# CSB5/lofreq

Measured on AMD Instinct MI355X. Metric: pileup columns/sec at depth 10000, higher is better.
Workload: dtype f64

## Files before the change

lofreq_amd/csrc/lfq_api.hip:

```cpp
#include "lfq_bound.h"
#include "lfq_ctx.h"

namespace {

struct LfqDeviceStreams {
    hipStream_t stream = nullptr, dps = nullptr, side[2] = {nullptr, nullptr};
    hipEvent_t ev_tail[3] = {nullptr, nullptr, nullptr};
    bool tail_recorded = false;
    hipEvent_t ev_end = nullptr;
    bool end_recorded = false;
    int refs = 0;
};
std::mutex g_streams_m;
LfqDeviceStreams g_streams[64];

bool acquire_streams(int device, lfq_ctx *c);
void release_streams(int device);

void *pin_acquire_impl(lfq_ctx *c, size_t bytes, int *slot)
{
    int best = -1, empty = -1, smallest = -1;
    for (int i = 0; i < LFQ_PIN_SLOTS; i++) {
        auto &b = c->pin_pool[i];
        if (b.used) {
// ... 576 lines not shown
                                   (LFQ_MAX_SEGMENTS + 1) * LFQ_NCOUNTERS * sizeof(int32_t), hipMemcpyDeviceToHost, st));
        LFQ_TRY_HIP(hipEventRecord(c->ev[3], st));
        c->batch_recorded = 1;
        return LFQ_OK;
    }

    int64_t max_depth = tr->max_col_obs;
    if (max_depth <= 0) {
        LFQ_TRY(lfq_launch_maxdepth(T, gcounters, st));
        LFQ_TRY_HIP(hipMemcpyAsync(c->h_counters, gcounters, LFQ_NCOUNTERS * sizeof(int32_t), hipMemcpyDeviceToHost, st));
        LFQ_TRY_HIP(hipStreamSynchronize(st));
        max_depth = c->h_counters[LFQ_GC_MAXDEPTH];
    }
    {
        static const LfqLuts h_luts = [] {
            LfqLuts h;
            fill_luts(&h);
            return h;
        }();
        const bool lb = !P.general && P.def_alt_bq == 0 && P.def_alt_jp < 0.0;
        P.bound_p_lo = (lb && !indel_mode && kn.bound_gate && lfq_count_is_lean(T, P, max_depth))
                           ? lfq_bound_p_lo(h_luts.bq, P.min_alt_bq4, LFQ_BOUND_QLO) : 0.0;
    }
    const int64_t per_block = 3 * max_depth + 72;
    int n_big_blocks = c->n_cu;
    const int64_t budget = (int64_t)1 << 29;
    if (per_block * n_big_blocks > budget) {
        n_big_blocks = (int)std::max<int64_t>(8, budget / per_block);
    }
    LFQ_TRY(grow(&c->d_scratch, &c->scratch_doubles, per_block * n_big_blocks));
    if (!c->d_longs) {
        c->long_cap = 1 << 16;
        c->pool_cells = kn.split_pool_cells;
        LFQ_TRY_HIP(hipMalloc((void **)&c->d_longs, (size_t)c->long_cap * sizeof(LfqLong)));
        LFQ_TRY_HIP(hipMalloc((void **)&c->d_pool, (size_t)std::max(c->pool_cells, 1) * sizeof(LfqSegCell)));
        LFQ_TRY_HIP(hipEventCreateWithFlags(&c->ev_segw, hipEventDisableTiming));
        LFQ_TRY_HIP(hipEventCreateWithFlags(&c->ev_prep, hipEventDisableTiming));
        LFQ_TRY_HIP(hipEventCreateWithFlags(&c->ev_mid, hipEventDisableTiming));
    }

    const int n_seg = 1;
    c->cur_segments = n_seg;
    LFQ_TRY_HIP(hipEventRecord(c->ev_join[2], st));
    LFQ_TRY_HIP(hipStreamWaitEvent(dps, c->ev_join[2], 0));

    bool big_joined = false;
    for (int s = 0; s < n_seg; s++) {
        const int64_t c0 = ncols * s / n_seg, c1 = ncols * (s + 1) / n_seg;
        LfqWork W;
        W.tested_prefix = c->d_prefix;
        W.entries = c->d_entries + c0;
        W.counters = c->d_counters + s * LFQ_NCOUNTERS;
        W.gcounters = gcounters;
        W.block_sums = (int32_t *)(c->d_tiles + 2 * (c0 / 1024 + 8 * s));
        W.long_cap = c->long_cap / n_seg;
        W.pool_cells = c->pool_cells / n_seg;
        W.longs = c->d_longs + (int64_t)s * W.long_cap;
        W.pool = c->d_pool + (int64_t)s * W.pool_cells;
        W.unsplit = c->d_unsplit + c0;

        LFQ_TRY_HIP(hipEventRecord(c->ev_cnt[s][0], st));
        const bool ungated = c->batch_gate == LFQ_GATE_NONE && st == c->stream && !c->priv_stream_on && !single_stream;
        LFQ_TRY(lfq_launch_count(T, c0, c1, P, c->d_luts, d_counts, c->d_flags, max_depth, st, ungated));
        c->cur_sparse_counts = P.sparse_counts && lfq_count_is_shallow(T, P, max_depth);
        LFQ_TRY_HIP(hipEventRecord(c->ev_cnt[s][1], st));

        LFQ_TRY_HIP(hipStreamWaitEvent(dps, c->ev_cnt[s][1], 0));
        LFQ_TRY(lfq_launch_scan(T, c0, c1, c->d_flags, d_counts, W, dps));
        if (P.approx_n > 0) {
            LFQ_TRY(grow(&c->d_approx_mu, &c->approx_mu_bytes, (c1 - c0) * 8));
            LFQ_TRY(lfq_launch_approx_gate(T, P, c->d_luts, d_counts, W, c1 - c0, (double *)c->d_approx_mu, c->d_flags, dps));
            LFQ_TRY(lfq_launch_scan(T, c0, c1, c->d_flags, d_counts, W, dps, true));
        }
        LFQ_TRY_HIP(hipEventRecord(c->ev_scan[s], dps));
        const bool sb_heavy = n_seg == 1 && !indel_mode && c->leader && !kn.no_sb_precompute;
        auto launch_heavy = [&]() -> int {
            if (P.lazy_strand) {
                LFQ_TRY(lfq_launch_strand_heavy(T, W, d_counts, c->d_tuples_mapped, c->d_nheavy_mapped, c->heavy_cap, 16, dps));
            } else {
                LFQ_TRY(lfq_launch_gather_heavy(W, d_counts, c->d_tuples_mapped, c->d_nheavy_mapped, c->heavy_cap, 16, dps));
            }
            LFQ_TRY_HIP(hipEventRecord(c->ev_heavy, dps));
            {
                std::lock_guard<std::mutex> lk(*c->lm);
                c->leader_go++;
                c->sb_pending++;
            }
            c->lcv->notify_all();
            return LFQ_OK;
        };
        const bool screen = !kn.skip_light && kn.light_kernel != 2;
        if (sb_heavy && !screen) {
            LFQ_TRY(launch_heavy());
        }
        const int64_t seg_cols = c1 - c0;
        const int screen_auto = (c->batch_gate == LFQ_GATE_NONE && !indel_mode) ? (tr->max_col_obs >= 4096 ? 1 : 2) : 4;
        const int light_waves_per_cu = kn.light_kernel == 0 ? screen_auto : 10;
        const int n_light_waves = (int)std::min<int64_t>((int64_t)c->n_cu * light_waves_per_cu, std::max<int64_t>(seg_cols / 8, 4));
        const int n_mid_waves = (int)std::min<int64_t>((int64_t)c->n_cu * 4, std::max<int64_t>(seg_cols, 4));
        const bool run_big = !kn.skip_big, run_mid = !kn.skip_mid;
        const bool dbg_sync = kn.debug_sync != 0;
#define LFQ_DBG_STAGE(name)                                                        \
    do {                                                                           \
        if (dbg_sync) {                                                            \
            fprintf(stderr, "[lfq] %s launched\n", name);                          \
            hipError_t e_ = hipDeviceSynchronize();                                \
            fprintf(stderr, "[lfq] %s done (%d)\n", name, (int)e_);                \
        }                                                                          \
    } while (0)
        LFQ_TRY_HIP(hipStreamWaitEvent(side1, c->ev_scan[s], 0));
        LFQ_TRY_HIP(hipEventRecord(c->ev_side[1][s][0], side1));
        LFQ_TRY_HIP(hipStreamWaitEvent(side0, c->ev_scan[s], 0));
        LFQ_TRY_HIP(hipEventRecord(c->ev_side[0][s][0], side0));
        if (run_big) {
            LFQ_TRY(lfq_launch_dp_big_prep(T, P, c->d_luts, d_counts, W, d_pvals, pvals_capacity, c->n_cu * 2, side0));
            LFQ_DBG_STAGE("prep");
        }
        LFQ_TRY_HIP(hipEventRecord(c->ev_prep, side0));
        if (run_mid) {
            LFQ_TRY(lfq_launch_dp_mid(T, P, c->d_luts, d_counts, W, d_pvals, pvals_capacity, n_mid_waves, side1));
            LFQ_DBG_STAGE("mid");
        }
        const bool big_on_st = run_big && !single_stream && !kn.big_on_side && c->batch_gate != LFQ_GATE_NONE;
        if (big_on_st) {
            LFQ_TRY_HIP(hipStreamWaitEvent(st, c->ev_prep, 0));
            LFQ_TRY(lfq_launch_dp_big(T, P, c->d_luts, d_counts, W, d_pvals, pvals_capacity, c->d_scratch, per_block,
                                      n_big_blocks, st));
            LFQ_DBG_STAGE("big");
            LFQ_TRY_HIP(hipEventRecord(c->ev_segw, st));
            big_joined = true;
        }
        if (run_big) {
            LFQ_TRY(lfq_launch_dp_seg(1, T, P, c->d_luts, W, c->n_cu * 8, side0));
            LFQ_DBG_STAGE("seg big");
            LFQ_TRY(tail_record(c, 0, side0));
            LFQ_TRY(lfq_launch_dp_combine(1, P, d_counts, W, d_pvals, pvals_capacity, c->n_cu, side0));
            LFQ_DBG_STAGE("combine big");
            if (!big_on_st) {
                LFQ_TRY(lfq_launch_dp_big(T, P, c->d_luts, d_counts, W, d_pvals, pvals_capacity, c->d_scratch, per_block,
                                          n_big_blocks, side0));
                LFQ_DBG_STAGE("big");
            }
        }
        if (!run_big) {
            LFQ_TRY(tail_record(c, 0, side0));
        }
        LFQ_TRY_HIP(hipStreamWaitEvent(side1, c->ev_prep, 0));
        if (run_mid || run_big) {
            LFQ_TRY(lfq_launch_dp_seg(0, T, P, c->d_luts, W, c->n_cu * 8, side1));
            LFQ_DBG_STAGE("seg mid");
            LFQ_TRY(tail_record(c, 1, side1));
            LFQ_TRY(lfq_launch_dp_combine(0, P, d_counts, W, d_pvals, pvals_capacity, c->n_cu, side1));
            LFQ_DBG_STAGE("combine mid");
        }
        if (!(run_mid || run_big)) {
            LFQ_TRY(tail_record(c, 1, side1));
        }
        LFQ_TRY_HIP(hipEventRecord(c->ev_light[s][0], dps));
        if (!kn.skip_light) {
            if (kn.light_kernel == 2) {
                LFQ_TRY(lfq_launch_dp_light(T, P, c->d_luts, d_counts, W, d_pvals, pvals_capacity, n_light_waves, dps));
            } else {
                const int kh = indel_mode ? c->kreg_hint_indel : c->kreg_hint;
                LFQ_TRY(lfq_launch_dp_quad(T, P, c->d_luts, d_counts, W, c->d_retry + c0, d_pvals, pvals_capacity,
                                           n_light_waves, kh, dps, 1));
                LFQ_TRY(tail_record(c, 2, dps));
                if (sb_heavy) {
                    LFQ_TRY(launch_heavy());
                }
                LFQ_TRY(lfq_launch_dp_quad(T, P, c->d_luts, d_counts, W, c->d_retry + c0, d_pvals, pvals_capacity,
                                           n_light_waves, kh, dps, 2));
            }
        }
        LFQ_TRY_HIP(hipEventRecord(c->ev_light[s][1], dps));
        if (!screen) {
            LFQ_TRY(tail_record(c, 2, dps));
        }
        for (int i = 0; i < 2; i++) {
            LFQ_TRY_HIP(hipEventRecord(c->ev_side[i][s][1], side_i[i]));
        }
    }
    hipStream_t jn = (st != c->stream || single_stream) ? st : side0;
// ... 760 lines not shown
```

lofreq_amd/csrc/lfq_dp.hip:

```cpp
#include <atomic>

#include "lfq_bound.h"
#include "lfq_device.h"

#define LFQ_LN2_HI 6.93147180369123816490e-01
#define LFQ_LN2_LO 1.90821492927058770002e-10
#define LFQ_EXP_UNDERFLOW_X (-708.3964185322641)
#define LFQ_DBL_EPS 2.220446049250313e-16

#ifndef LFQ_HEAVY_WAVES
#define LFQ_HEAVY_WAVES 8
#endif
#ifndef LFQ_DP512_WAVES
#define LFQ_DP512_WAVES 2
#endif

struct LfqColCtx {
    int col;
    uint64_t off0;
    int64_t n_obs;
    int ref_code;
    int median_ref_bq;
    int K;
    int64_t bonf;
// ... 363 lines not shown
template <int C>
__device__ __forceinline__ void lfq_strip_store_cells(const LfqStrip<C> &S, int gl, int shift, int K, LfqSegCell *out)
{
#pragma unroll
    for (int j = 0; j < C; j++) {
        const int k = gl * C + j - shift;
        if (k >= 0 && k <= K && (k < K || j == 0)) {
            const double v = S.v[j];
            LfqSegCell c;
            c.v = (v > 0.0) ? __builtin_amdgcn_frexp_mant(v) : 0.0;
            c.e = (v > 0.0) ? S.e + __builtin_amdgcn_frexp_exp(v) : LFQ_EXT_ZERO_E;
            c.pad_ = 0;
            out[k] = c;
        }
    }
}

__device__ __forceinline__ int lfq_split_plan(int K, int64_t rem_chunks, int phase1, int seg_max)
{
    if (K > LFQ_SPLIT_MAX_K) {
        return 0;
    }
    int64_t n_new = seg_max - phase1;
    n_new = min(n_new, rem_chunks / (rem_chunks < LFQ_SEG_SHORT_BELOW ? LFQ_SEG_MIN_CHUNKS_SHORT : LFQ_SEG_MIN_CHUNKS));
    n_new = min(n_new, max(rem_chunks * 64 / (2 * (int64_t)max(K, 1)) + 1 - phase1, (int64_t)3 - phase1));
    return n_new >= 2 ? (int)n_new : 0;
}

__device__ __forceinline__ int lfq_seg_class(int K)
{
    return K <= 63 ? 0 : (K <= 252 ? 1 : (K <= 504 ? 2 : (K <= 1008 ? 3 : 4)));
}

__device__ __forceinline__ LfqLong *lfq_long_reserve(const LfqWork &W, int K, int n_seg, int64_t *cell0)
{
    const int cells = 2 * n_seg * (K + 1);
    const int c0 = atomicAdd(&W.counters[LFQ_CNT_POOL], cells);
    if (c0 + cells > W.pool_cells) {
        return nullptr;
    }
    const int cls = lfq_seg_class(K);
    const int per_class = W.long_cap / LFQ_SEG_CLASSES;
    const int slot = atomicAdd(&W.counters[LFQ_CNT_LONG0 + cls], 1);
    if (slot >= per_class) {
        return nullptr;
    }
    *cell0 = c0;
    return W.longs + cls * per_class + slot;
}

__device__ __forceinline__ void lfq_ctx_from_long(LfqColCtx &cx, const LfqLong &r, const LfqParams &P)
{
    cx.col = r.col;
    cx.off0 = r.off0;
    cx.n_obs = r.n_obs;
    cx.ref_code = r.ref_code;
    cx.median_ref_bq = r.median_ref_bq;
    cx.K = r.K;
    cx.bonf = r.bonf;
    cx.bonf_d = (double)r.bonf;
    cx.sig_s = P.sig * (1.0 + P.prune_slack);
    if (r.force_fe) {
        cx.sig_s = fmax(cx.sig_s, 4.5e-16 * cx.bonf_d);
    }
}

__device__ __forceinline__ void lfq_seg_range(const LfqLong &rec, int r, int64_t *c0, int64_t *c1)
{
    const int64_t n_chunks = ((int64_t)rec.n_obs + 63) / 64;
    const int64_t rem = n_chunks - rec.ch_begin;
    const int n_new = rec.n_seg - rec.phase1;
    *c0 = rec.ch_begin + rem * (r - rec.phase1) / n_new;
    *c1 = rec.ch_begin + rem * (r - rec.phase1 + 1) / n_new;
}

__device__ __forceinline__ double lfq_logaddexp(double a, double b)
{
    const double hi = fmax(a, b), lo = fmin(a, b);
    if (lo == -INFINITY) {
// ... 281 lines not shown
            }
            if (pf.want_entry) {
                *pf.entry = lfq_load_entry(pf.entry_ptr, 0);
            }
        }
        if (PREFETCH && ch + 1 < n_chunks) {
            raw = lfq_load_chunk(cx, ch + 1, T);
        }
#ifdef LFQ_PROFILE
        const long long c2 = clock64();
        t_load += c2 - c1;
#endif
        const bool hit = lfq_strip_chunk2<C>(S, reinterpret_cast<const LfqRow2 *>(rows), tflag, lt, cx.bonf_d, cx.sig_s);
#ifdef LFQ_PROFILE
        t_rows += clock64() - c2;
#endif
        n_rows += __popcll(S.rows >= 64 ? km : (km & ((1ull << S.rows) - 1ull)));
        if (hit) {
            pruned = true;
            break;
        }
        if (SPLIT && ch + 1 == P.phase1_chunks) {
            const int n_new = lfq_split_plan(K, n_chunks - (ch + 1), 1,
                                             min(P.seg_max_mid, max(2, P.seg_budget_mid / max(W.counters[LFQ_CNT_MID], 1))));
            if (n_new > 0) {
                const int n_seg = n_new + 1;
                const int cells = 2 * n_seg * (K + 1);
                const int cls = lfq_seg_class(K);
                const int per_class = W.long_cap / LFQ_SEG_CLASSES;
                const int c0 = lfq_claim(&W.counters[LFQ_CNT_POOL], cells);
                if (c0 + cells <= W.pool_cells) {
                    const int slot = lfq_claim(&W.counters[LFQ_CNT_LONG0 + cls], 1);
                    if (slot < per_class) {
                        lfq_strip_store_cells<C>(S, lane, shift, K, W.pool + c0);
                        if (lane == 0) {
                            LfqLong r;
                            r.off0 = cx.off0;
                            r.bonf = cx.bonf;
                            r.cell0 = c0;
                            r.n_obs = (int32_t)cx.n_obs;
                            r.col = cx.col;
                            r.K = K;
                            r.n_seg = n_seg;
                            r.ch_begin = (int32_t)(ch + 1);
                            r.phase1 = 1;
                            r.uf_mask = 0;
                            r.force_fe = 0;
                            r.pruned = 0;
                            r.rows = n_rows;
                            r.median_ref_bq = (int16_t)cx.median_ref_bq;
                            r.ref_code = (uint8_t)cx.ref_code;
                            r.pad0_ = 0;
                            r.pad1_ = 0;
                            r.uf_bound[0] = r.uf_bound[1] = r.uf_bound[2] = 0.0;
                            r.pad_[0] = r.pad_[1] = r.pad_[2] = r.pad_[3] = 0;
                            W.longs[cls * per_class + slot] = r;
                        }
                        return;
                    }
                }
            }
        }
        if (!PREFETCH && ch + 1 < n_chunks) {
            raw = lfq_load_chunk(cx, ch + 1, T);
        }
    }
#ifdef LFQ_PROFILE
    if (lane == 0) {
        atomicAdd(&W.counters[8], (int)(t_stage >> 8));
        atomicAdd(&W.counters[9], (int)(t_load >> 8));
        atomicAdd(&W.counters[10], (int)(t_rows >> 8));
        atomicAdd(&W.counters[11], n_rows);
    }
#endif
#ifdef LFQ_TRACE
    if (lane == 0) printf("col %d K %d C %d: rows done pruned=%d n_rows=%d\n", cx.col, K, C, (int)pruned, n_rows);
#endif
    if (lane == 0) {
        lfq_account(W, n_rows, K);
    }
    if (!pruned && !lfq_strip_final_prune<C>(S, lt, cx.bonf_d, cx.sig_s)) {
#ifdef LFQ_TRACE
        if (lane == 0) printf("col %d: emitting\n", cx.col);
#endif
        const lfq_col_counts cnt = counts[cx.col];
        S.rows = n_rows;
        lfq_emit_linear<C>(cx, cnt, S, shift, lt, W, pvals, pvals_capacity);
    }
}

template <int MAXC>
__global__ __launch_bounds__(256) void lfq_dp_wave_kernel(LfqTracksDev T, LfqParams P,
                                                          const LfqLuts *__restrict__ g_luts,
                                                          const lfq_col_counts *__restrict__ counts, LfqWork W,
                                                          int base_idx, int count_idx,
                                                          lfq_col_pvals *__restrict__ pvals,
                                                          int64_t pvals_capacity, int batch, int only_if_gl64)
{
    __shared__ LfqLuts s_luts;
    __shared__ LfqRow s_rows[4][64];
    (void)only_if_gl64;
    if (MAXC > 1) {
        __builtin_amdgcn_s_setprio(3);
    }
    lfq_luts_to_lds(&s_luts, g_luts);
    __syncthreads();
    const int wave = __builtin_amdgcn_readfirstlane((int)(threadIdx.x >> 6));
    const int n_work = W.counters[count_idx];
    const LfqEntry *list = W.entries + ((base_idx >= 0) ? W.counters[base_idx] : 0);
    LfqRow *rows = s_rows[wave];

    const int BATCH = batch;
    int32_t *head = &W.counters[(MAXC == 1) ? LFQ_CNT_HEAD_LIGHT : LFQ_CNT_HEAD_MID];
    for (;;) {
        int b0 = lfq_claim(head, BATCH);
        if (b0 >= n_work) {
            break;
        }
        const int b1 = min(b0 + BATCH, n_work);
        int w = b0;
        LfqEntry en = lfq_load_entry(list, w);
        LfqRaw raw = lfq_load_chunk_at(en.off0, en.n_obs, 0, T);
        LfqEntry en_next = en;
        bool have_next = (w + 1) < b1;
        if (have_next) {
            en_next = lfq_load_entry(list, w + 1);
        }
        for (;;) {
            LfqColCtx cx;
            lfq_col_setup(cx, en, P);
            LfqRaw raw_next = raw;
            LfqEntry en_next2 = en_next;
            const bool have_next2 = have_next && (w + 2) < b1;
            LfqPrefetch pf;
            pf.want_raw = have_next;
            pf.off0 = en_next.off0;
            pf.n_obs = en_next.n_obs;
            pf.want_entry = have_next2;
            pf.entry_ptr = list + (have_next2 ? (w + 2) : w);
            pf.raw = &raw_next;
            pf.entry = &en_next2;
            if (MAXC == 1 || cx.K < 64) {
                lfq_wave_column<1, (MAXC > 1), (MAXC > 1)>(cx, raw, T, P, &s_luts, rows, counts, W, pvals, pvals_capacity, pf);
            } else {
                lfq_wave_column<4, true, true>(cx, raw, T, P, &s_luts, rows, counts, W, pvals, pvals_capacity, pf);
            }
            if (!have_next) {
                break;
// ... 611 lines not shown
                                                 LfqSegCell *out)
{
    const int lane = lfq_lane();
    const int K = cx.K;
    const int shift = (C - K % C) % C;
    const int lt = (K + shift) / C;
    const double tflag = (lane == lt) ? 1.0 : 0.0;
    LfqStrip<C> S;
    lfq_strip_init<C>(S, true, shift);
    bool pruned = false;
    int n_rows = 0;
    LfqRaw raw = lfq_load_chunk(cx, ch0, T);
    for (int64_t ch = ch0; ch < ch1; ch++) {
        const uint64_t km = lfq_stage_rows2(cx, raw, P, L, reinterpret_cast<LfqRow2 *>(rows));
        if (ch + 1 < ch1) {
            raw = lfq_load_chunk(cx, ch + 1, T);
        }
        const bool hit = lfq_strip_chunk2<C>(S, reinterpret_cast<const LfqRow2 *>(rows), tflag, lt, cx.bonf_d, cx.sig_s);
        n_rows += __popcll(S.rows >= 64 ? km : (km & ((1ull << S.rows) - 1ull)));
        if (hit) {
            pruned = true;
            break;
        }
    }
    if (!pruned && lfq_strip_final_prune<C>(S, lt, cx.bonf_d, cx.sig_s)) {
        pruned = true;
    }
    lfq_strip_store_cells<C>(S, lane, shift, K, out);
    if (lane == 0) {
        __builtin_nontemporal_store(n_rows | (pruned ? (int)0x40000000 : 0), &out[0].pad_);
    }
}

template <int MODE>
__global__ __launch_bounds__(256) void lfq_dp_seg_kernel(LfqTracksDev T, LfqParams P,
                                                         const LfqLuts *__restrict__ g_luts, LfqWork W)
{
    __shared__ LfqLuts s_luts;
    __shared__ LfqRow s_rows[4][64];
    __builtin_amdgcn_s_setprio(3);
    lfq_luts_to_lds(&s_luts, g_luts);
    __syncthreads();
    constexpr int C_LO = MODE ? 2 : 0, C_N = MODE ? 3 : 2;
    const int wave = __builtin_amdgcn_readfirstlane((int)(threadIdx.x >> 6));
    const int per_class = W.long_cap / LFQ_SEG_CLASSES;
    int n_items[C_N], total = 0;
#pragma unroll
    for (int c = 0; c < C_N; c++) {
        n_items[c] = min(W.counters[LFQ_CNT_LONG0 + C_LO + c], per_class) * LFQ_SEG_MAX;
        total += n_items[c];
    }
    LfqRow *rows = s_rows[wave];
    const int n_waves_total = (int)gridDim.x * 4;
    for (int idx = (int)blockIdx.x * 4 + wave; idx < total; idx += n_waves_total) {
        int c = 0, i = idx;
#pragma unroll
        for (int k = 0; k < C_N - 1; k++) {
            if (c == k && i >= n_items[k]) {
                i -= n_items[k];
                c = k + 1;
            }
        }
        const int r = i % LFQ_SEG_MAX;
        const LfqLong R = W.longs[(C_LO + c) * per_class + i / LFQ_SEG_MAX];
        if (r < R.phase1 || r >= R.n_seg) {
            continue;
        }
        LfqColCtx cx;
        lfq_ctx_from_long(cx, R, P);
        int64_t c0, c1;
        lfq_seg_range(R, r, &c0, &c1);
        LfqSegCell *out = W.pool + R.cell0 + (int64_t)r * (R.K + 1);
        if (MODE == 0) {
            if (c == 0) {
                lfq_wave_segment<1>(cx, c0, c1, T, P, &s_luts, rows, out);
            } else {
                lfq_wave_segment<4>(cx, c0, c1, T, P, &s_luts, rows, out);
            }
        } else {
            if (c == 0) {
                lfq_wave_segment<8>(cx, c0, c1, T, P, &s_luts, rows, out);
            } else if (c == 1) {
                lfq_wave_segment<16>(cx, c0, c1, T, P, &s_luts, rows, out);
            } else {
                lfq_wave_segment<32>(cx, c0, c1, T, P, &s_luts, rows, out);
            }
        }
    }
}


#ifndef LFQ_COMB_THREADS
#define LFQ_COMB_THREADS 512
#endif
#define LFQ_FOLD_MAX_CLASS 3
#define LFQ_COMB_CELLS 2048
#define LFQ_COMB_PER_THREAD (LFQ_COMB_CELLS / LFQ_COMB_THREADS)

struct LfqCombShared {
    double av[LFQ_COMB_CELLS];
// ... 894 lines not shown
        atomicAdd(&W.gcounters[LFQ_GC_APPROX_PRUNED], 1);
    }
}

int lfq_launch_approx_gate(const LfqTracksDev &t, const LfqParams &p, const LfqLuts *d_luts, const lfq_col_counts *d_counts,
                           const LfqWork &w, int64_t ncols_seg, double *d_mu, uint8_t *d_flags, void *stream)
{
    if (ncols_seg <= 0) {
        return LFQ_OK;
    }
    const unsigned waves = (unsigned)std::min<int64_t>(ncols_seg, 256 * 32);
    hipLaunchKernelGGL(lfq_approx_mu_kernel, dim3((waves + 3) / 4), dim3(256), 0, (hipStream_t)stream, t, p, d_luts, d_counts,
                       w, d_mu);
    hipLaunchKernelGGL(lfq_approx_gate_kernel, dim3((unsigned)((ncols_seg + 255) / 256)), dim3(256), 0, (hipStream_t)stream,
                       p, w, (const double *)d_mu, d_flags);
    return hipGetLastError() == hipSuccess ? LFQ_OK : LFQ_ERR_HIP;
}

int lfq_launch_dp_light(const LfqTracksDev &t, const LfqParams &p, const LfqLuts *d_luts,
                        const lfq_col_counts *d_counts, const LfqWork &w, lfq_col_pvals *d_pvals,
                        int64_t pvals_capacity, int n_waves, void *stream)
{
    if (t.ncols <= 0 || n_waves <= 0) {
        return LFQ_OK;
    }
    const unsigned blocks = (unsigned)((n_waves + 3) / 4);
    hipLaunchKernelGGL(lfq_dp_wave_kernel<1>, dim3(blocks), dim3(256), 0, (hipStream_t)stream, t, p, d_luts,
                       d_counts, w, -1, LFQ_CNT_LIGHT, d_pvals, pvals_capacity, 32, 0);
    return hipGetLastError() == hipSuccess ? LFQ_OK : LFQ_ERR_HIP;
}

int lfq_launch_dp_mid(const LfqTracksDev &t, const LfqParams &p, const LfqLuts *d_luts,
                      const lfq_col_counts *d_counts, const LfqWork &w, lfq_col_pvals *d_pvals,
                      int64_t pvals_capacity, int n_waves, void *stream)
{
    if (t.ncols <= 0 || n_waves <= 0) {
        return LFQ_OK;
    }
    const unsigned blocks = (unsigned)((n_waves + 3) / 4);
    hipLaunchKernelGGL(lfq_dp_wave_kernel<4>, dim3(blocks), dim3(256), 0, (hipStream_t)stream, t, p,
                       d_luts, d_counts, w, LFQ_CNT_LIGHT, LFQ_CNT_MID, d_pvals, pvals_capacity, 1, 0);
    return hipGetLastError() == hipSuccess ? LFQ_OK : LFQ_ERR_HIP;
}

int lfq_launch_dp_big(const LfqTracksDev &t, const LfqParams &p, const LfqLuts *d_luts,
                      const lfq_col_counts *d_counts, const LfqWork &w, lfq_col_pvals *d_pvals,
                      int64_t pvals_capacity, double *d_scratch, int64_t scratch_doubles_per_block,
                      int n_blocks, void *stream)
{
    if (t.ncols <= 0 || n_blocks <= 0) {
        return LFQ_OK;
    }
    hipLaunchKernelGGL(lfq_dp_big_kernel, dim3((unsigned)n_blocks), dim3(LFQ_HEAVY_WAVES * 64), 0,
                       (hipStream_t)stream, t, p, d_luts, d_counts, w, d_pvals, pvals_capacity, d_scratch,
                       scratch_doubles_per_block);
    return hipGetLastError() == hipSuccess ? LFQ_OK : LFQ_ERR_HIP;
}


int lfq_launch_dp_big_prep(const LfqTracksDev &t, const LfqParams &p, const LfqLuts *d_luts,
                           const lfq_col_counts *d_counts, const LfqWork &w, lfq_col_pvals *d_pvals,
                           int64_t pvals_capacity, int n_blocks, void *stream)
{
    if (t.ncols <= 0 || n_blocks <= 0) {
        return LFQ_OK;
    }
    hipLaunchKernelGGL(lfq_dp_big_prep_kernel, dim3((unsigned)n_blocks), dim3(LFQ_PREP_WAVES * 64), 0,
                       (hipStream_t)stream, t, p, d_luts, d_counts, w, d_pvals, pvals_capacity);
    return hipGetLastError() == hipSuccess ? LFQ_OK : LFQ_ERR_HIP;
}

int lfq_launch_dp_seg(int mode, const LfqTracksDev &t, const LfqParams &p, const LfqLuts *d_luts,
                      const LfqWork &w, int n_waves, void *stream)
{
    if (t.ncols <= 0 || n_waves <= 0) {
        return LFQ_OK;
    }
    const dim3 grid((unsigned)((n_waves + 3) / 4)), block(256);
    if (mode == 0) {
        hipLaunchKernelGGL(lfq_dp_seg_kernel<0>, grid, block, 0, (hipStream_t)stream, t, p, d_luts, w);
    } else {
        hipLaunchKernelGGL(lfq_dp_seg_kernel<1>, grid, block, 0, (hipStream_t)stream, t, p, d_luts, w);
    }
    return hipGetLastError() == hipSuccess ? LFQ_OK : LFQ_ERR_HIP;
}

int lfq_launch_dp_combine(int mode, const LfqParams &p, const lfq_col_counts *d_counts, const LfqWork &w,
                          lfq_col_pvals *d_pvals, int64_t pvals_capacity, int n_blocks, void *stream)
{
    if (n_blocks <= 0) {
        return LFQ_OK;
    }
    {
        static std::atomic<unsigned long long> allowed{0ull};
        int dev = 0;
        if (hipGetDevice(&dev) != hipSuccess) {
            return LFQ_ERR_HIP;
        }
        const unsigned long long bit = 1ull << (dev & 63);
        if (!(allowed.load(std::memory_order_acquire) & bit)) {
            const int bytes = (int)sizeof(LfqCombShared);
            if (hipFuncSetAttribute(reinterpret_cast<const void *>(&lfq_dp_combine_kernel<0>),
                                    hipFuncAttributeMaxDynamicSharedMemorySize, bytes) != hipSuccess ||
                hipFuncSetAttribute(reinterpret_cast<const void *>(&lfq_dp_combine_kernel<1>),
                                    hipFuncAttributeMaxDynamicSharedMemorySize, bytes) != hipSuccess) {
                return LFQ_ERR_HIP;
            }
            allowed.fetch_or(bit, std::memory_order_release);
        }
    }
    if (mode == 0) {
        hipLaunchKernelGGL(lfq_dp_fold_kernel<0>, dim3((unsigned)n_blocks * 4), dim3(64 * LFQ_FOLD_WAVES), 0,
                           (hipStream_t)stream, p, d_counts, w, d_pvals, pvals_capacity);
        hipLaunchKernelGGL(lfq_dp_combine_kernel<0>, dim3((unsigned)n_blocks), dim3(LFQ_COMB_THREADS), sizeof(LfqCombShared),
                           (hipStream_t)stream, p, d_counts, w, d_pvals, pvals_capacity, 1);
    } else {
// ... 57 lines not shown
```

lofreq_amd/csrc/lfq_host.cpp:

```cpp
#include <errno.h>
#include <fenv.h>
#include <float.h>
#include <limits.h>
#include <math.h>
#include <stdio.h>
#include <stdlib.h>
#include <string.h>

#include <algorithm>
#include <atomic>
#include <chrono>
#include <condition_variable>
#include <functional>
#include <mutex>
#include <sched.h>
#include <string>
#include <thread>
#include <unordered_map>
#include <vector>

#include "lofreq_amd.h"
#include "lfq_internal.h"

#ifdef LFQ_TUNE
// ... 23 lines not shown
        x.host_loop_threads = geti("LFQ_HOST_LOOP_THREADS", 8);
        x.host_spin_us = geti("LFQ_HOST_SPIN_US", 2000);
        x.local_world_size = (int)std::max(1L, geti("LOCAL_WORLD_SIZE", 1));
        x.no_sb_precompute = LFQ_TUNE_HAS("LFQ_NO_SB_PRECOMPUTE");
#ifdef LFQ_TUNE
        if (const char *sk = getenv("LFQ_DEBUG_SKIP")) {
            x.skip_light = strstr(sk, "light") != nullptr;
            x.skip_mid = strstr(sk, "mid") != nullptr;
            x.skip_big = strstr(sk, "big") != nullptr;
        }
        if (const char *lk = getenv("LFQ_LIGHT_KERNEL")) {
            x.light_kernel = !strcmp(lk, "wave") ? 2 : 0;
        }
#endif
        x.screen_rounds = (int)std::max(1L, LFQ_TUNE_I("LFQ_SCREEN_ROUNDS", 24));
        {
            const long both = LFQ_TUNE_I("LFQ_SEG_MAX", -1);
            const long big = LFQ_TUNE_I("LFQ_SEG_MAX_BIG", both), mid = LFQ_TUNE_I("LFQ_SEG_MAX_MID", both);
            x.seg_max = big < 0 ? -1 : (int)std::min((long)LFQ_SEG_MAX, std::max(2L, big));
            x.seg_max_mid = mid < 0 ? -1 : (int)std::min((long)LFQ_SEG_MAX, std::max(2L, mid));
        }
        x.split_pool_cells = (int)std::max(0L, LFQ_TUNE_I("LFQ_SPLIT_POOL_CELLS", 8L << 20));
        x.count_multi_below = LFQ_TUNE_I("LFQ_COUNT_MULTI_BELOW", 4096);
        x.big_on_side = LFQ_TUNE_HAS("LFQ_BIG_ON_SIDE");
        x.pileup_tiles = (int)LFQ_TUNE_I("LFQ_PILEUP_TILES", 1);
        x.baq_one_variant = LFQ_TUNE_HAS("LFQ_BAQ_ONE_VARIANT") ? 1 : 0;
        x.count_lpg4_below = LFQ_TUNE_I("LFQ_COUNT_LPG4_BELOW", 320);
        x.count_lpg8_below = LFQ_TUNE_I("LFQ_COUNT_LPG8_BELOW", 900);
        x.host_par_min = std::max(1L, LFQ_TUNE_I("LFQ_HOST_PAR_MIN", 200000));
        x.indel_host_pack = LFQ_TUNE_HAS("LFQ_INDEL_HOST_PACK");
        x.pileup_atomic = LFQ_TUNE_HAS("LFQ_PILEUP_ATOMIC");
        x.baq_lds = LFQ_TUNE_I("LFQ_BAQ_LDS", 1) != 0;
        x.bound_gate = LFQ_TUNE_I("LFQ_BOUND_GATE", 1) != 0;
        (void)geti;
        (void)has;
        return x;
    }();
    return k;
}

namespace {

inline double phred_to_prob(int q)
{
    return (q == INT_MAX) ? DBL_MIN : pow(10.0, -1.0 * q / 10.0);
}

inline int prob_to_phred(long double p) { return (int)(-10.0 * log10l(p)); }

inline int prob_to_phred_safe(double p) { return (p <= 0.0) ? INT_MAX : (int)(-10.0 * log10l(p)); }

inline int eps_cmp(double a, double b)
{
    if (fabs(a - b) < DBL_EPSILON) {
        return 0;
    }
    return a < b ? -1 : (a > b ? 1 : 0);
}

struct IndexedP {
    double p;
    int64_t i;
};

void sort_indexed(std::vector<IndexedP> &v)
{
// ... 1268 lines not shown
```

lofreq_amd/csrc/lfq_internal.h:

```cpp
#ifndef LFQ_INTERNAL_H
#define LFQ_INTERNAL_H

#include <stdint.h>

#include "lofreq_amd.h"

struct LfqLuts {
    double bq[256];
    double baq[256];
    double mq[256];
    double sq[256];
};

struct LfqParams {
    int32_t min_bq4;
    int32_t min_alt_bq4;
    int32_t def_alt_bq;
    int32_t general;
    double jq_reject_above;
    double alt_jq_reject_above;
    double def_alt_jp;
    int32_t min_cov;
    int32_t use_baq, use_mq, use_sq;
    int32_t bonf_dynamic;
// ... 36 lines not shown
    int32_t pad2_;
};

#define LFQ_FLAG_NLO_SHIFT 3

struct LfqSegCell {
    double v;
    int32_t e;
    int32_t pad_;
};

struct LfqLong {
    uint64_t off0;
    int64_t bonf;
    int64_t cell0;
    int32_t n_obs, col;
    int32_t K;
    int32_t n_seg;
    int32_t ch_begin;
    int32_t phase1;
    uint32_t uf_mask;
    int32_t force_fe;
    int32_t pruned;
    int32_t rows;
    int16_t median_ref_bq;
    uint8_t ref_code;
    uint8_t pad0_;
    int32_t pad1_;
    double uf_bound[3];
    int64_t pad_[4];
};

#define LFQ_SEG_MAX 8
#define LFQ_SEG_CLASSES 5
#define LFQ_SEG_MIN_CHUNKS 16
#ifndef LFQ_SEG_MIN_CHUNKS_SHORT
#define LFQ_SEG_MIN_CHUNKS_SHORT 4
#endif
#define LFQ_SEG_SHORT_BELOW 48
#define LFQ_PHASE1_CHUNKS 8
#define LFQ_SEG_BUDGET 4096
#define LFQ_SPLIT_MAX_K 2016

#if defined(__HIPCC__)
__host__ __device__
#endif
static inline int lfq_khist_thr(int f)
{
    return f == 0 ? 5 : f == 1 ? 7 : f == 2 ? 9 : f == 3 ? 11 : f == 4 ? 15 : f == 5 ? 23 : 31;
}

struct LfqWork {
    int32_t *tested_prefix;
    LfqEntry *entries;
    int32_t *gcounters;
    int32_t *counters;
    int32_t *block_sums;
    LfqLong *longs;
    int32_t *unsplit;
    LfqSegCell *pool;
    int32_t long_cap;
    int32_t pool_cells;
};

#define LFQ_MID_K 64
#define LFQ_BIG_K 250
#define LFQ_NCOUNTERS 320
#define LFQ_MAX_SEGMENTS 1
#define LFQ_GC_PVALS 0
#define LFQ_GC_OVERFLOW 1
#define LFQ_GC_TESTED 2
#define LFQ_GC_MAXDEPTH 3
#define LFQ_GC_CELLS 8
#define LFQ_GC_ROWS 10
#define LFQ_GC_APPROX_PRUNED 13
#define LFQ_GC_SCREEN_RETRY 12
#define LFQ_CNT_TESTED 0
#define LFQ_CNT_BIG 1
#define LFQ_CNT_MID 2
#define LFQ_CNT_LIGHT 3
#define LFQ_CNT_HEAD 4
#define LFQ_CNT_CARRY_IN 15
#define LFQ_CNT_HEAD_LIGHT 12
#define LFQ_CNT_HEAD_MID 13
#define LFQ_CNT_UNSPLIT 5
#define LFQ_CNT_HEAD_PREP 6
#define LFQ_CNT_POOL 7
#define LFQ_CNT_HEAD_COMB 24
#define LFQ_CNT_HEAD_FOLD 48
#define LFQ_CNT_KLE7 26
#define LFQ_CNT_KLE15 27
#define LFQ_CNT_KLE31 28
#define LFQ_CNT_XHEAD 64
#define LFQ_CNT_KHIST 40
#define LFQ_NKHIST 7
#define LFQ_CNT_LONG0 16

#define LFQ_SEQ_LETTERS "ACGTN=MRSVWYHKDB"
#if defined(__HIPCC__)
__host__ __device__
#endif
static inline char lfq_seq_letter(unsigned code)
{
    return code > 15u ? 'N' : LFQ_SEQ_LETTERS[code];
}

struct LfqKnobs {
    int timing;
    int single_stream;
    int no_sb_precompute;
    int debug_sync;
    int skip_light, skip_mid, skip_big;
    int light_kernel;
    int screen_rounds;
    int seg_max;
    int seg_max_mid;
    int split_pool_cells;
    long count_multi_below;
    int big_on_side;
    int baq_one_variant;
    int pileup_tiles;
    long host_loop_threads;
    long count_lpg4_below, count_lpg8_below;
    long host_spin_us;
    int sync_upload;
    int host_threads;
    long host_par_min;
    int local_world_size;
    int indel_host_pack;
    int pileup_atomic;
    int baq_lds;
    long baq_scratch_mb;
    int private_stream;
    int bound_gate;
};
const LfqKnobs &lfq_knobs(void);
unsigned lfq_cpu_budget(void);

void lfq_sb_precompute(const int32_t *tuples, int64_t n);

static inline int64_t lfq_al(int64_t b)
{
    return (b + 255) / 256 * 256;
}

struct LfqReadsDev {
    int64_t n_reads;
    const int32_t *pos;
    const int64_t *cigar_off, *seq_off;
    const uint32_t *cigar;
    const uint8_t *seq, *qual;
    const uint8_t *baq;
    const uint8_t *mapq, *reverse;
    const uint8_t *ref;
    int64_t ref_len;
    const uint8_t *sq;
    const uint8_t *bi, *bd;
    const uint8_t *tag_flags;
    const int32_t *pmax_end;
    const int32_t *read_idx;
};

struct LfqBaqGeom {
    int32_t xb, l_ref;
    int32_t bw;
};
struct LfqBaqRead {
// ... 142 lines not shown
    int32_t nonmatch_qual, min_bq;
    double *scratch;
    int64_t scratch_cells;
    double *prob;
    uint8_t *status;
};
int lfq_launch_srcq(const LfqSrcqArgs &a, const LfqLuts *d_luts, int n_blocks, void *stream);
int lfq_launch_pileup_scatter(const LfqPileupArgs &a, void *stream);

int lfq_launch_strand_heavy(const LfqTracksDev &t, const LfqWork &w, lfq_col_counts *d_counts, int32_t *tuples_mapped,
                            int32_t *n_mapped, int cap_entries, int min_alt, void *stream);
int lfq_launch_strand_pvals(const LfqTracksDev &t, lfq_col_pvals *d_pvals, const int32_t *d_n_pvals, int64_t cap, int n_blocks,
                            void *stream);
int lfq_launch_gather_heavy(const LfqWork &w, const lfq_col_counts *d_counts, int32_t *tuples_mapped,
                            int32_t *n_mapped, int cap_entries, int min_alt, void *stream);
int lfq_launch_maxdepth(const LfqTracksDev &t, int32_t *d_gcounters, void *stream);
int lfq_launch_ntcount(const LfqTracksDev &t, int32_t *d_out, void *stream);
bool lfq_count_is_shallow(const LfqTracksDev &t, const LfqParams &p, int64_t max_col_obs);
int lfq_launch_count(const LfqTracksDev &t, int64_t c0, int64_t c1, const LfqParams &p, const LfqLuts *d_luts,
                     lfq_col_counts *d_counts, uint8_t *d_flags, int64_t max_col_obs, void *stream, bool shallow_half_cu = false);
bool lfq_count_is_lean(const LfqTracksDev &t, const LfqParams &p, int64_t max_col_obs);
int lfq_launch_scan(const LfqTracksDev &t, int64_t c0, int64_t c1, const uint8_t *d_flags,
                    const lfq_col_counts *d_counts, const LfqWork &w, void *stream, bool relist = false);
int lfq_launch_approx_gate(const LfqTracksDev &t, const LfqParams &p, const LfqLuts *d_luts, const lfq_col_counts *d_counts,
                           const LfqWork &w, int64_t ncols_seg, double *d_mu, uint8_t *d_flags, void *stream);
int lfq_launch_dp_light(const LfqTracksDev &t, const LfqParams &p, const LfqLuts *d_luts,
                        const lfq_col_counts *d_counts, const LfqWork &w, lfq_col_pvals *d_pvals,
                        int64_t pvals_capacity, int n_waves, void *stream);
int lfq_launch_dp_quad(const LfqTracksDev &t, const LfqParams &p, const LfqLuts *d_luts,
                       const lfq_col_counts *d_counts, const LfqWork &w, uint8_t *d_retry, lfq_col_pvals *d_pvals,
                       int64_t pvals_capacity, int n_waves, int kreg_hint, void *stream, int phase = 0);
int lfq_launch_dp_mid(const LfqTracksDev &t, const LfqParams &p, const LfqLuts *d_luts,
                      const lfq_col_counts *d_counts, const LfqWork &w, lfq_col_pvals *d_pvals,
                      int64_t pvals_capacity, int n_waves, void *stream);
int lfq_launch_dp_big(const LfqTracksDev &t, const LfqParams &p, const LfqLuts *d_luts,
                      const lfq_col_counts *d_counts, const LfqWork &w, lfq_col_pvals *d_pvals,
                      int64_t pvals_capacity, double *d_scratch, int64_t scratch_doubles_per_block,
                      int n_blocks, void *stream);
int lfq_launch_dp_big_prep(const LfqTracksDev &t, const LfqParams &p, const LfqLuts *d_luts,
                           const lfq_col_counts *d_counts, const LfqWork &w, lfq_col_pvals *d_pvals,
                           int64_t pvals_capacity, int n_blocks, void *stream);
int lfq_launch_dp_seg(int mode, const LfqTracksDev &t, const LfqParams &p, const LfqLuts *d_luts,
                      const LfqWork &w, int n_waves, void *stream);
int lfq_launch_dp_combine(int mode, const LfqParams &p, const lfq_col_counts *d_counts, const LfqWork &w,
                          lfq_col_pvals *d_pvals, int64_t pvals_capacity, int n_blocks, void *stream);
int lfq_launch_synth(const struct lfq_synth_spec *d_spec_host, int64_t col_begin, int64_t ncols,
                     uint8_t *d_nt, uint8_t *d_bq, uint8_t *d_baq, uint8_t *d_mq, uint64_t *d_col_off,
                     uint8_t *d_ref_base, int nt_packed, void *stream);

#endif
```

Measured before the change: 370.5 million.

## Compact segment work items into a list and make DP workgroup size configurable

The long-column reserve paths now append packed (class, slot, segment) items to a per-mode compacted list stored after the long records. The segment kernel iterates only over these items instead of scanning every class slot times LFQ_SEG_MAX and skipping empty ones, and blocks beyond the item count exit before loading the lookup tables. The mid-DP and segment kernels are also templated on waves per workgroup, selectable through an environment knob that defaults to 4. The cost is an extra atomic counter claim and item stores on the reserve path, plus a larger allocation for the long records.

```diff
diff --git a/lofreq_amd/csrc/lfq_api.hip b/lofreq_amd/csrc/lfq_api.hip
--- a/lofreq_amd/csrc/lfq_api.hip
+++ b/lofreq_amd/csrc/lfq_api.hip
@@ -632,7 +632,7 @@
     if (!c->d_longs) {
         c->long_cap = 1 << 16;
         c->pool_cells = kn.split_pool_cells;
-        LFQ_TRY_HIP(hipMalloc((void **)&c->d_longs, (size_t)c->long_cap * sizeof(LfqLong)));
+        LFQ_TRY_HIP(hipMalloc((void **)&c->d_longs, (size_t)c->long_cap * (sizeof(LfqLong) + LFQ_SEG_MAX * sizeof(int32_t))));
         LFQ_TRY_HIP(hipMalloc((void **)&c->d_pool, (size_t)std::max(c->pool_cells, 1) * sizeof(LfqSegCell)));
         LFQ_TRY_HIP(hipEventCreateWithFlags(&c->ev_segw, hipEventDisableTiming));
         LFQ_TRY_HIP(hipEventCreateWithFlags(&c->ev_prep, hipEventDisableTiming));
@@ -698,6 +698,7 @@
         const int light_waves_per_cu = kn.light_kernel == 0 ? screen_auto : 10;
         const int n_light_waves = (int)std::min<int64_t>((int64_t)c->n_cu * light_waves_per_cu, std::max<int64_t>(seg_cols / 8, 4));
         const int n_mid_waves = (int)std::min<int64_t>((int64_t)c->n_cu * 4, std::max<int64_t>(seg_cols, 4));
+        const int dp_wg = (c->batch_gate == LFQ_GATE_NONE && !indel_mode && kn.dp_wg_waves > 0) ? kn.dp_wg_waves : 4;
         const bool run_big = !kn.skip_big, run_mid = !kn.skip_mid;
         const bool dbg_sync = kn.debug_sync != 0;
 #define LFQ_DBG_STAGE(name)                                                        \
@@ -718,7 +719,7 @@
         }
         LFQ_TRY_HIP(hipEventRecord(c->ev_prep, side0));
         if (run_mid) {
-            LFQ_TRY(lfq_launch_dp_mid(T, P, c->d_luts, d_counts, W, d_pvals, pvals_capacity, n_mid_waves, side1));
+            LFQ_TRY(lfq_launch_dp_mid(T, P, c->d_luts, d_counts, W, d_pvals, pvals_capacity, n_mid_waves, dp_wg, side1));
             LFQ_DBG_STAGE("mid");
         }
         const bool big_on_st = run_big && !single_stream && !kn.big_on_side && c->batch_gate != LFQ_GATE_NONE;
@@ -731,7 +732,7 @@
             big_joined = true;
         }
         if (run_big) {
-            LFQ_TRY(lfq_launch_dp_seg(1, T, P, c->d_luts, W, c->n_cu * 8, side0));
+            LFQ_TRY(lfq_launch_dp_seg(1, T, P, c->d_luts, W, c->n_cu * 8, dp_wg, side0));
             LFQ_DBG_STAGE("seg big");
             LFQ_TRY(tail_record(c, 0, side0));
             LFQ_TRY(lfq_launch_dp_combine(1, P, d_counts, W, d_pvals, pvals_capacity, c->n_cu, side0));
@@ -747,7 +748,7 @@
         }
         LFQ_TRY_HIP(hipStreamWaitEvent(side1, c->ev_prep, 0));
         if (run_mid || run_big) {
-            LFQ_TRY(lfq_launch_dp_seg(0, T, P, c->d_luts, W, c->n_cu * 8, side1));
+            LFQ_TRY(lfq_launch_dp_seg(0, T, P, c->d_luts, W, c->n_cu * 8, dp_wg, side1));
             LFQ_DBG_STAGE("seg mid");
             LFQ_TRY(tail_record(c, 1, side1));
             LFQ_TRY(lfq_launch_dp_combine(0, P, d_counts, W, d_pvals, pvals_capacity, c->n_cu, side1));
diff --git a/lofreq_amd/csrc/lfq_dp.hip b/lofreq_amd/csrc/lfq_dp.hip
--- a/lofreq_amd/csrc/lfq_dp.hip
+++ b/lofreq_amd/csrc/lfq_dp.hip
@@ -419,6 +419,11 @@
     return K <= 63 ? 0 : (K <= 252 ? 1 : (K <= 504 ? 2 : (K <= 1008 ? 3 : 4)));
 }
 
+__device__ __forceinline__ int32_t *lfq_seg_items_of(const LfqWork &W)
+{
+    return reinterpret_cast<int32_t *>(W.longs + W.long_cap);
+}
+
 __device__ __forceinline__ LfqLong *lfq_long_reserve(const LfqWork &W, int K, int n_seg, int64_t *cell0)
 {
     const int cells = 2 * n_seg * (K + 1);
@@ -432,6 +437,8 @@
     if (slot >= per_class) {
         return nullptr;
     }
+    const int item0 = atomicAdd(&W.counters[LFQ_CNT_SEG_ITEMS + lfq_seg_mode_of(cls)], n_seg);
+    lfq_seg_items_put(lfq_seg_items_of(W), per_class, item0, cls, slot, 0, n_seg, 0, 1);
     *cell0 = c0;
     return W.longs + cls * per_class + slot;
 }
@@ -779,6 +786,8 @@
                 if (c0 + cells <= W.pool_cells) {
                     const int slot = lfq_claim(&W.counters[LFQ_CNT_LONG0 + cls], 1);
                     if (slot < per_class) {
+                        const int item0 = lfq_claim(&W.counters[LFQ_CNT_SEG_ITEMS + lfq_seg_mode_of(cls)], n_new);
+                        lfq_seg_items_put(lfq_seg_items_of(W), per_class, item0, cls, slot, 1, n_seg, lane, 64);
                         lfq_strip_store_cells<C>(S, lane, shift, K, W.pool + c0);
                         if (lane == 0) {
                             LfqLong r;
@@ -836,16 +845,17 @@
     }
 }
 
-template <int MAXC>
-__global__ __launch_bounds__(256) void lfq_dp_wave_kernel(LfqTracksDev T, LfqParams P,
-                                                          const LfqLuts *__restrict__ g_luts,
-                                                          const lfq_col_counts *__restrict__ counts, LfqWork W,
-                                                          int base_idx, int count_idx,
-                                                          lfq_col_pvals *__restrict__ pvals,
-                                                          int64_t pvals_capacity, int batch, int only_if_gl64)
+template <int MAXC, int WG = 4>
+__global__ __launch_bounds__(WG * 64) void lfq_dp_wave_kernel(LfqTracksDev T, LfqParams P,
+                                                              const LfqLuts *__restrict__ g_luts,
+                                                              const lfq_col_counts *__restrict__ counts, LfqWork W,
+                                                              int base_idx, int count_idx,
+                                                              lfq_col_pvals *__restrict__ pvals,
+                                                              int64_t pvals_capacity, int batch, int only_if_gl64)
 {
     __shared__ LfqLuts s_luts;
-    __shared__ LfqRow s_rows[4][64];
+    __shared__ LfqRow s_rows[WG][64];
+    __shared__ int s_first;
     (void)only_if_gl64;
     if (MAXC > 1) {
         __builtin_amdgcn_s_setprio(3);
@@ -859,8 +869,19 @@
 
     const int BATCH = batch;
     int32_t *head = &W.counters[(MAXC == 1) ? LFQ_CNT_HEAD_LIGHT : LFQ_CNT_HEAD_MID];
-    for (;;) {
-        int b0 = lfq_claim(head, BATCH);
+    int b_first = 0;
+    if (WG > 4) {
+        if (wave == 0) {
+            const int b = lfq_claim(head, WG * BATCH);
+            if (lfq_lane() == 0) {
+                s_first = b;
+            }
+        }
+        __syncthreads();
+        b_first = __builtin_amdgcn_readfirstlane(s_first) + wave * BATCH;
+    }
+    for (bool first = true;; first = false) {
+        int b0 = (WG > 4 && first) ? b_first : lfq_claim(head, BATCH);
         if (b0 >= n_work) {
             break;
         }
@@ -1538,40 +1559,30 @@
     }
 }
 
-template <int MODE>
-__global__ __launch_bounds__(256) void lfq_dp_seg_kernel(LfqTracksDev T, LfqParams P,
-                                                         const LfqLuts *__restrict__ g_luts, LfqWork W)
+template <int MODE, int WG>
+__global__ __launch_bounds__(WG * 64) void lfq_dp_seg_kernel(LfqTracksDev T, LfqParams P,
+                                                             const LfqLuts *__restrict__ g_luts, LfqWork W)
 {
     __shared__ LfqLuts s_luts;
-    __shared__ LfqRow s_rows[4][64];
+    __shared__ LfqRow s_rows[WG][64];
+    constexpr int C_LO = MODE ? LFQ_SEG_MODE0_CLASSES : 0;
+    const int per_class = W.long_cap / LFQ_SEG_CLASSES;
+    const int total = W.counters[LFQ_CNT_SEG_ITEMS + MODE];
+    if ((int)blockIdx.x * WG >= total) {
+        return;
+    }
     __builtin_amdgcn_s_setprio(3);
     lfq_luts_to_lds(&s_luts, g_luts);
     __syncthreads();
-    constexpr int C_LO = MODE ? 2 : 0, C_N = MODE ? 3 : 2;
     const int wave = __builtin_amdgcn_readfirstlane((int)(threadIdx.x >> 6));
-    const int per_class = W.long_cap / LFQ_SEG_CLASSES;
-    int n_items[C_N], total = 0;
-#pragma unroll
-    for (int c = 0; c < C_N; c++) {
-        n_items[c] = min(W.counters[LFQ_CNT_LONG0 + C_LO + c], per_class) * LFQ_SEG_MAX;
-        total += n_items[c];
-    }
+    const int32_t *items = lfq_seg_items_of(W) + lfq_seg_items_base(MODE, per_class);
     LfqRow *rows = s_rows[wave];
-    const int n_waves_total = (int)gridDim.x * 4;
-    for (int idx = (int)blockIdx.x * 4 + wave; idx < total; idx += n_waves_total) {
-        int c = 0, i = idx;
-#pragma unroll
-        for (int k = 0; k < C_N - 1; k++) {
-            if (c == k && i >= n_items[k]) {
-                i -= n_items[k];
-                c = k + 1;
-            }
-        }
-        const int r = i % LFQ_SEG_MAX;
-        const LfqLong R = W.longs[(C_LO + c) * per_class + i / LFQ_SEG_MAX];
-        if (r < R.phase1 || r >= R.n_seg) {
-            continue;
-        }
+    const int n_waves_total = (int)gridDim.x * WG;
+    for (int idx = (int)blockIdx.x * WG + wave; idx < total; idx += n_waves_total) {
+        int cls, slot, r, rec;
+        lfq_seg_item_unpack(__builtin_amdgcn_readfirstlane(items[idx]), per_class, &cls, &slot, &r, &rec);
+        const int c = cls - C_LO;
+        const LfqLong R = W.longs[rec];
         LfqColCtx cx;
         lfq_ctx_from_long(cx, R, P);
         int64_t c0, c1;
@@ -2532,14 +2543,26 @@
 
 int lfq_launch_dp_mid(const LfqTracksDev &t, const LfqParams &p, const LfqLuts *d_luts,
                       const lfq_col_counts *d_counts, const LfqWork &w, lfq_col_pvals *d_pvals,
-                      int64_t pvals_capacity, int n_waves, void *stream)
+                      int64_t pvals_capacity, int n_waves, int wg_waves, void *stream)
 {
     if (t.ncols <= 0 || n_waves <= 0) {
         return LFQ_OK;
     }
-    const unsigned blocks = (unsigned)((n_waves + 3) / 4);
-    hipLaunchKernelGGL(lfq_dp_wave_kernel<4>, dim3(blocks), dim3(256), 0, (hipStream_t)stream, t, p,
-                       d_luts, d_counts, w, LFQ_CNT_LIGHT, LFQ_CNT_MID, d_pvals, pvals_capacity, 1, 0);
+    if (wg_waves != 4 && wg_waves != 8 && wg_waves != 16) {
+        return LFQ_ERR_INVALID;
+    }
+    const dim3 grid((unsigned)((n_waves + wg_waves - 1) / wg_waves)), block(64u * wg_waves);
+#define LFQ_LAUNCH_MID(WG)                                                                                          \
+    hipLaunchKernelGGL((lfq_dp_wave_kernel<4, WG>), grid, block, 0, (hipStream_t)stream, t, p, d_luts, d_counts, w, \
+                       LFQ_CNT_LIGHT, LFQ_CNT_MID, d_pvals, pvals_capacity, 1, 0)
+    if (wg_waves == 4) {
+        LFQ_LAUNCH_MID(4);
+    } else if (wg_waves == 8) {
+        LFQ_LAUNCH_MID(8);
+    } else {
+        LFQ_LAUNCH_MID(16);
+    }
+#undef LFQ_LAUNCH_MID
     return hipGetLastError() == hipSuccess ? LFQ_OK : LFQ_ERR_HIP;
 }
 
@@ -2571,17 +2594,31 @@
 }
 
 int lfq_launch_dp_seg(int mode, const LfqTracksDev &t, const LfqParams &p, const LfqLuts *d_luts,
-                      const LfqWork &w, int n_waves, void *stream)
+                      const LfqWork &w, int n_waves, int wg_waves, void *stream)
 {
     if (t.ncols <= 0 || n_waves <= 0) {
         return LFQ_OK;
     }
-    const dim3 grid((unsigned)((n_waves + 3) / 4)), block(256);
-    if (mode == 0) {
-        hipLaunchKernelGGL(lfq_dp_seg_kernel<0>, grid, block, 0, (hipStream_t)stream, t, p, d_luts, w);
+    if (wg_waves != 4 && wg_waves != 8 && wg_waves != 16) {
+        return LFQ_ERR_INVALID;
+    }
+    const dim3 grid((unsigned)((n_waves + wg_waves - 1) / wg_waves)), block(64u * wg_waves);
+#define LFQ_LAUNCH_SEG(WG)                                                                                          \
+    do {                                                                                                            \
+        if (mode == 0) {                                                                                            \
+            hipLaunchKernelGGL((lfq_dp_seg_kernel<0, WG>), grid, block, 0, (hipStream_t)stream, t, p, d_luts, w);   \
+        } else {                                                                                                    \
+            hipLaunchKernelGGL((lfq_dp_seg_kernel<1, WG>), grid, block, 0, (hipStream_t)stream, t, p, d_luts, w);   \
+        }                                                                                                           \
+    } while (0)
+    if (wg_waves == 4) {
+        LFQ_LAUNCH_SEG(4);
+    } else if (wg_waves == 8) {
+        LFQ_LAUNCH_SEG(8);
     } else {
-        hipLaunchKernelGGL(lfq_dp_seg_kernel<1>, grid, block, 0, (hipStream_t)stream, t, p, d_luts, w);
-    }
+        LFQ_LAUNCH_SEG(16);
+    }
+#undef LFQ_LAUNCH_SEG
     return hipGetLastError() == hipSuccess ? LFQ_OK : LFQ_ERR_HIP;
 }
 
diff --git a/lofreq_amd/csrc/lfq_host.cpp b/lofreq_amd/csrc/lfq_host.cpp
--- a/lofreq_amd/csrc/lfq_host.cpp
+++ b/lofreq_amd/csrc/lfq_host.cpp
@@ -79,6 +79,10 @@
         x.pileup_atomic = LFQ_TUNE_HAS("LFQ_PILEUP_ATOMIC");
         x.baq_lds = LFQ_TUNE_I("LFQ_BAQ_LDS", 1) != 0;
         x.bound_gate = LFQ_TUNE_I("LFQ_BOUND_GATE", 1) != 0;
+        {
+            const long w = LFQ_TUNE_I("LFQ_DP_WG_WAVES", 0);
+            x.dp_wg_waves = w <= 0 ? 0 : (w >= 16 ? 16 : (w >= 8 ? 8 : 4));
+        }
         (void)geti;
         (void)has;
         return x;
diff --git a/lofreq_amd/csrc/lfq_internal.h b/lofreq_amd/csrc/lfq_internal.h
--- a/lofreq_amd/csrc/lfq_internal.h
+++ b/lofreq_amd/csrc/lfq_internal.h
@@ -92,6 +92,7 @@
 };
 
 #define LFQ_SEG_MAX 8
+#include "lfq_seg_items.h"
 #define LFQ_SEG_CLASSES 5
 #define LFQ_SEG_MIN_CHUNKS 16
 #ifndef LFQ_SEG_MIN_CHUNKS_SHORT
@@ -155,6 +156,7 @@
 #define LFQ_CNT_KHIST 40
 #define LFQ_NKHIST 7
 #define LFQ_CNT_LONG0 16
+#define LFQ_CNT_SEG_ITEMS 22
 
 #define LFQ_SEQ_LETTERS "ACGTN=MRSVWYHKDB"
 #if defined(__HIPCC__)
@@ -193,6 +195,7 @@
     long baq_scratch_mb;
     int private_stream;
     int bound_gate;
+    int dp_wg_waves;
 };
 const LfqKnobs &lfq_knobs(void);
 unsigned lfq_cpu_budget(void);
@@ -401,7 +404,7 @@
                        int64_t pvals_capacity, int n_waves, int kreg_hint, void *stream, int phase = 0);
 int lfq_launch_dp_mid(const LfqTracksDev &t, const LfqParams &p, const LfqLuts *d_luts,
                       const lfq_col_counts *d_counts, const LfqWork &w, lfq_col_pvals *d_pvals,
-                      int64_t pvals_capacity, int n_waves, void *stream);
+                      int64_t pvals_capacity, int n_waves, int wg_waves, void *stream);
 int lfq_launch_dp_big(const LfqTracksDev &t, const LfqParams &p, const LfqLuts *d_luts,
                       const lfq_col_counts *d_counts, const LfqWork &w, lfq_col_pvals *d_pvals,
                       int64_t pvals_capacity, double *d_scratch, int64_t scratch_doubles_per_block,
@@ -410,7 +413,7 @@
                            const lfq_col_counts *d_counts, const LfqWork &w, lfq_col_pvals *d_pvals,
                            int64_t pvals_capacity, int n_blocks, void *stream);
 int lfq_launch_dp_seg(int mode, const LfqTracksDev &t, const LfqParams &p, const LfqLuts *d_luts,
-                      const LfqWork &w, int n_waves, void *stream);
+                      const LfqWork &w, int n_waves, int wg_waves, void *stream);
 int lfq_launch_dp_combine(int mode, const LfqParams &p, const lfq_col_counts *d_counts, const LfqWork &w,
                           lfq_col_pvals *d_pvals, int64_t pvals_capacity, int n_blocks, void *stream);
 int lfq_launch_synth(const struct lfq_synth_spec *d_spec_host, int64_t col_begin, int64_t ncols,
diff --git a/lofreq_amd/csrc/lfq_seg_items.h b/lofreq_amd/csrc/lfq_seg_items.h
--- /dev/null
+++ b/lofreq_amd/csrc/lfq_seg_items.h
@@ -0,0 +1,49 @@
+#ifndef LFQ_SEG_ITEMS_H
+#define LFQ_SEG_ITEMS_H
+
+#include <stdint.h>
+
+#if defined(__HIPCC__)
+#define LFQ_SEG_HD __host__ __device__
+#else
+#define LFQ_SEG_HD
+#endif
+
+#ifndef LFQ_SEG_MAX
+#define LFQ_SEG_MAX 8
+#endif
+#define LFQ_SEG_MODE0_CLASSES 2
+
+LFQ_SEG_HD static inline int lfq_seg_mode_of(int cls)
+{
+    return cls >= LFQ_SEG_MODE0_CLASSES ? 1 : 0;
+}
+
+LFQ_SEG_HD static inline int lfq_seg_items_base(int mode, int per_class)
+{
+    return mode ? LFQ_SEG_MODE0_CLASSES * per_class * LFQ_SEG_MAX : 0;
+}
+
+LFQ_SEG_HD static inline int32_t lfq_seg_item_pack(int cls, int slot, int r, int per_class)
+{
+    return (int32_t)((cls * per_class + slot) * LFQ_SEG_MAX + r);
+}
+
+LFQ_SEG_HD static inline void lfq_seg_item_unpack(int32_t item, int per_class, int *cls, int *slot, int *r, int *rec)
+{
+    *r = item % LFQ_SEG_MAX;
+    *rec = item / LFQ_SEG_MAX;
+    *cls = *rec / per_class;
+    *slot = *rec % per_class;
+}
+
+LFQ_SEG_HD static inline void lfq_seg_items_put(int32_t *table, int per_class, int item0, int cls, int slot, int phase1,
+                                                int n_seg, int first, int step)
+{
+    int32_t *list = table + lfq_seg_items_base(lfq_seg_mode_of(cls), per_class);
+    for (int j = first; j < n_seg - phase1; j += step) {
+        list[item0 + j] = lfq_seg_item_pack(cls, slot, phase1 + j, per_class);
+    }
+}
+
+#endif
diff --git a/lofreq_amd/csrc/lfq_seg_items_check.cpp b/lofreq_amd/csrc/lfq_seg_items_check.cpp
--- /dev/null
+++ b/lofreq_amd/csrc/lfq_seg_items_check.cpp
@@ -0,0 +1,61 @@
+#include <stdio.h>
+#include <stdlib.h>
+
+#include <vector>
+
+#include "lfq_seg_items.h"
+
+#define N_CLASSES 5
+
+int main(void)
+{
+    char line[256];
+    while (fgets(line, sizeof(line), stdin)) {
+        if (line[0] == '\n' || line[0] == '#') {
+            continue;
+        }
+        long per_class = 0, n = 0;
+        if (sscanf(line, "S %ld %ld", &per_class, &n) != 2 || per_class < 1 || per_class > 4096 || n < 0) {
+            return 2;
+        }
+        std::vector<int32_t> table((size_t)N_CLASSES * (size_t)per_class * LFQ_SEG_MAX, -1);
+        int n_cls[N_CLASSES] = {0, 0, 0, 0, 0}, n_items[2] = {0, 0};
+        for (long i = 0; i < n; i++) {
+            int cls = 0, n_seg = 0, phase1 = 0;
+            if (!fgets(line, sizeof(line), stdin) || sscanf(line, "%d %d %d", &cls, &n_seg, &phase1) != 3 || cls < 0
+                || cls >= N_CLASSES || phase1 < 0 || phase1 > 1 || n_seg - phase1 < 1 || n_seg > LFQ_SEG_MAX) {
+                return 2;
+            }
+            const int slot = n_cls[cls]++;
+            if (slot >= per_class) {
+                continue;
+            }
+            const int mode = lfq_seg_mode_of(cls);
+            const int item0 = n_items[mode];
+            n_items[mode] += n_seg - phase1;
+            if (phase1) {
+                for (int lane = 0; lane < 64; lane++) {
+                    lfq_seg_items_put(table.data(), (int)per_class, item0, cls, slot, phase1, n_seg, lane, 64);
+                }
+            } else {
+                lfq_seg_items_put(table.data(), (int)per_class, item0, cls, slot, phase1, n_seg, 0, 1);
+            }
+        }
+        for (int mode = 0; mode < 2; mode++) {
+            const int base = lfq_seg_items_base(mode, (int)per_class);
+            const int end = mode ? (int)table.size() : lfq_seg_items_base(1, (int)per_class);
+            int stray = 0;
+            for (int i = base + n_items[mode]; i < end; i++) {
+                stray += table[(size_t)i] != -1;
+            }
+            printf("M %d %d %d\n", mode, n_items[mode], stray);
+            for (int i = 0; i < n_items[mode]; i++) {
+                int cls, slot, r, rec;
+                lfq_seg_item_unpack(table[(size_t)(base + i)], (int)per_class, &cls, &slot, &r, &rec);
+                printf("I %d %d %d %d %d %d\n", mode, i, cls, slot, r, rec);
+            }
+        }
+        printf("E\n");
+    }
+    return 0;
+}
```

New measurement: 381.9 million, median of 6. 3.1% higher.
